# klemens-floege/oneprot

Measured on AMD Instinct MI355X. Metric: protein-pairs/sec/node (seq+struct-token, L=512, ESM-2-150M), higher is better.
Workload: dtype bf16; 1 GPU; cfg-2: seq<->struct_token sub-step, facebook/esm2_t30_150M_UR50D / facebook/esm2_t30_150M_UR50D, L=512, 256 pairs/GPU per modality, global batch 256, output_dim 1024, CLIP local_loss+gather_with_grad, L1 0.01, Adam 1e-3, clip 1.0, sequence encoder frozen (reference default), random-init weights; global_batch=256, seq_len=512, parallelism=dp1, frozen_sequence_encoder=True

## Files before the change

include/oneprot_hip.h:

```cpp
#ifndef ONEPROT_HIP_H
#define ONEPROT_HIP_H
#include <stddef.h>
#include <stdint.h>
#ifdef __cplusplus
extern "C" {
#endif

int oneprot_abi_version(void);

int oneprot_esm_embed_fwd(const int64_t* ids, const float* table, float* x, float* row_scale, int B, int L, int d, int vocab,
                          int pad_id, int mask_id, int token_dropout, void* stream);
size_t oneprot_esm_embed_bwd_workspace(int T, int d, int vocab);
int oneprot_esm_embed_bwd(const int64_t* ids, const float* dx, const float* row_scale, float* dtable, void* workspace, int B, int L, int d,
                          int vocab, int pad_id, int mask_id, int token_dropout, int accumulate, void* stream);
int oneprot_bert_embed_fwd(const int64_t* ids, const float* word, const float* pos, const float* type0, const float* gamma, const float* beta,
                           float* x_f32, void* x_bf16, int B, int L, int d, int vocab, float eps, void* stream);

int oneprot_layernorm_fwd(const void* x, int x_is_bf16, const float* gamma, const float* beta, void* y_bf16, float* y_f32, float* mean,
                          float* rstd, int64_t T, int d, float eps, void* stream);
size_t oneprot_layernorm_bwd_workspace(int d);
int oneprot_layernorm_bwd(const void* dy, int dy_mode, const float* wrow, int L, const void* x, int x_is_bf16, const float* gamma,
                          const float* mean, const float* rstd, const float* add_to, float* dx, void* dx_bf16 ,
                          float* dgamma, float* dbeta, void* workspace, int64_t T, int d, int accumulate_param_grads, void* stream);
int oneprot_lnpool_fwd(const float* x, const int64_t* ids, int pad_id, const float* gamma, const float* beta, float* pooled, float* mean,
// ... 33 lines not shown
int oneprot_sched_late_draws(const void* sched_ws);
int64_t oneprot_sched_epoch(const void* sched_ws);
int oneprot_gemm_resid_ln8_eligible(int64_t M, int N, int K);
int oneprot_gemm_resid_ln8_error(const void* sched_ws);
int oneprot_gemm_resid_ln8_error_clear(void* sched_ws, void* stream);
void oneprot_gemm_resid_ln8_poll_bound(int polls);
int oneprot_gemm_bf16_nt_resid_ln8(const void* A, const void* W, int64_t M, int N, int K, int lda, int ldb, const float* bias, const float* resid,
                                   float* x_out, const float* gamma, const float* beta, float eps, void* h_bf16, float* stats, void* sched_ws,
                                   size_t sched_ws_bytes, void* stream);
void oneprot_gemm_ln_form(int form);
int oneprot_gemm_ln_form_get(void);
void oneprot_gemm_force_shape(int shape);
void oneprot_gemm_tune(int sup_m, int sup_n);
size_t oneprot_gemm_bf16_tn_workspace(int N, int K);
void oneprot_gemm_tn_variant(int v);
void oneprot_cu_reserve(int cus);
int oneprot_gemm_bf16_tn(const void* dY, const void* X, int64_t M, int N, int K, int ldy, int ldx, float* dW, float* dbias, void* workspace,
                         size_t workspace_bytes, int accumulate, void* stream);
int oneprot_sgemm(const float* A, const float* B, float* C, int M, int N, int K, int transA, int b_is_kn, float alpha, int accumulate, void* stream);

int oneprot_attn_fwd(const void* q, const void* k, const void* v, const float* key_bias, void* ctx, float* lse, int B, int H, int L, int hd,
                     void* stream);
size_t oneprot_attn_bwd_workspace(int B, int H, int L);
int oneprot_attn_bwd(const void* q, const void* k, const void* v, const float* key_bias, const void* ctx, const void* dctx, const float* lse,
                     const float* rope_cos, const float* rope_sin, float q_scale, void* dqkv, void* workspace, int B, int H, int L, int hd,
                     void* stream);
int oneprot_attn_fwd_dropout(const void* q, const void* k, const void* v, const float* key_bias, void* ctx, float* lse, int B, int H, int L, int hd,
                             float p, uint64_t seed, uint64_t stream_id, void* stream);
int oneprot_attn_bwd_dropout(const void* q, const void* k, const void* v, const float* key_bias, const void* ctx, const void* dctx, const float* lse,
                             const float* rope_cos, const float* rope_sin, float q_scale, void* dqkv, void* workspace, int B, int H, int L, int hd,
                             float p, uint64_t seed, uint64_t stream_id, void* stream);
int oneprot_attn_dropout_keep(void* keep, int B, int H, int L, float p, uint64_t seed, uint64_t stream_id, void* stream);
void oneprot_attn_force_bwd_path(int path);
void oneprot_attn_force_fwd_path(int path);

int oneprot_gelu_f32(const float* x, float* y, int64_t n, void* stream);
int oneprot_gelu_bwd_f32(const float* x, const float* dy, float* dx, int64_t n, void* stream);
int oneprot_l2norm_fwd(const float* x, float* y, float* inv_norm, int R, int D, float scale, void* stream);
int oneprot_l2norm_bwd(const float* y, const float* dy, const float* inv_norm, float* dx, int R, int D, float scale, float l1_coef, void* stream);
int oneprot_ce_fwd_bwd(float* logits, float* loss_sum, float* row_loss_ws , int R, int C, int label_offset, float row_weight, void* stream);
int oneprot_siglip_fwd_bwd(float* logits, float* loss_sum, float* row_loss_ws , int B, float logit_bias, int negative_only, void* stream);
int oneprot_siglip_fwd_bwd_dev(float* logits, float* loss_sum, float* row_loss_ws , int B, const float* logit_bias_dev, int negative_only, void* stream);
int oneprot_diag_rank(const float* logits, int* rank_row, int* rank_col, int N, void* stream);
int oneprot_abs_sum(const float* x, float* out_sum, void* workspace , int64_t n, float coef, void* stream);

int oneprot_dot_f32(const float* x, const float* y, float* out_sum, void* workspace , int64_t n, float coef, void* stream);

int oneprot_l1_bwd(const float* x, float* dx, int64_t n, float coef, const float* upstream, int accumulate, void* stream);
int oneprot_scale_by_device_scalar(float* x, int64_t n, const float* s, void* stream);
int oneprot_key_padding_bias(const int64_t* ids, float* bias, int64_t n, int pad_id, void* stream);

int oneprot_dropout_bf16(const void* x, void* y, int64_t n, float p, uint64_t seed, uint64_t stream_id, void* stream);
int oneprot_dropout_f32(const float* x, float* y, int64_t n, float p, uint64_t seed, uint64_t stream_id, void* stream);
int oneprot_dropout_add_f32(const float* x, const float* resid, float* y, int64_t n, float p, uint64_t seed, uint64_t stream_id, void* stream);
int oneprot_dropout_add_layernorm_fwd(const float* x, const float* resid, float* s_out, const float* gamma, const float* beta, void* y_bf16, float* y_f32,
                                      float* mean, float* rstd, int64_t T, int d, float eps, float p, uint64_t seed, uint64_t stream_id, void* stream);
int oneprot_dropout_bwd_add_bf16(const void* dy, void* dx, int64_t n, float p, uint64_t seed, uint64_t stream_id, void* stream);
int oneprot_dropout_bwd_add_f32(const void* dy, float* dx, int64_t n, float p, uint64_t seed, uint64_t stream_id, void* stream);

size_t oneprot_sumsq_workspace(void);
int oneprot_sumsq(const float* x, int64_t n, float* sumsq, void* workspace, void* stream);
int oneprot_clip_coef(const float* sumsq, float max_norm, float* coef, float* norm_out, const void* sched_ws , void* stream);
int oneprot_adam_step(float* p, const float* g, float* m, float* v, int64_t n, float lr, float beta1, float beta2, float eps, float weight_decay,
                      int step, const float* grad_scale, void* stream);

int oneprot_cast_f32_to_bf16(const float* src, void* dst, int64_t n, void* stream);
// ... 31 lines not shown
```

oneprot_amd/csrc/attention.hip:

```cpp
#include "common.h"
#include "sched_ws.h"
#include "../../include/oneprot_hip.h"
#include <float.h>
#include <atomic>
void* dynamic_tiles_workspace();

#define LOG2E 1.4426950408889634f
#define KC 256
#define RESCALE_THR 10.0f

template <int HD> struct Cfg {
  static constexpr int HDP = HD < 32 ? 32 : HD;
  static constexpr int NCH = HDP / 8;
  static constexpr int KSTEPS = HD / 16;
  static constexpr int DBLK = HDP / 32;
  static constexpr int ROWB = HDP * 2;
};

template <int HDP> __device__ __forceinline__ int swz(int row, int chunk) {
  return HDP == 32 ? (chunk ^ ((row >> 2) & 3)) : (chunk ^ ((row >> 1) & 7));
}

template <int HD> struct TileRegs { u32x4 v[KC * Cfg<HD>::NCH / 256]; };
template <int HD>
// ... 1312 lines not shown
  if (!q || !k || !v || !ctx || B <= 0 || H <= 0 || L <= 0) return OP_EINVAL;
  hipStream_t s = (hipStream_t)stream;
  if (g_attn_fwd_path != 0) {
    switch (hd) {
      case 16: return launch_fwd_nomax<16>(q, k, v, key_bias, ctx, lse, B, H, L, s);
      case 32: return launch_fwd_nomax<32>(q, k, v, key_bias, ctx, lse, B, H, L, s);
      case 64: return launch_fwd_nomax<64>(q, k, v, key_bias, ctx, lse, B, H, L, s);
      default: return OP_EINVAL;
    }
  }
  switch (hd) {
    case 16: return launch_fwd<16>(q, k, v, key_bias, ctx, lse, B, H, L, s);
    case 32: return launch_fwd<32>(q, k, v, key_bias, ctx, lse, B, H, L, s);
    case 64: return launch_fwd<64>(q, k, v, key_bias, ctx, lse, B, H, L, s);
    default: return OP_EINVAL;
  }
}

extern "C" int oneprot_attn_fwd_dropout(const void* q, const void* k, const void* v, const float* key_bias, void* ctx, float* lse, int B, int H, int L, int hd, float p,
                                        uint64_t seed, uint64_t stream_id, void* stream) {
  AttnDrop dr;
  if (!q || !k || !v || !ctx || B <= 0 || H <= 0 || L <= 0 || attn_drop_make(p, seed, stream_id, dr) != OP_OK) return OP_EINVAL;
  hipStream_t s = (hipStream_t)stream;
  switch (hd) {
    case 16: return launch_fwd_dropout<16>(q, k, v, key_bias, ctx, lse, B, H, L, dr, s);
    case 32: return launch_fwd_dropout<32>(q, k, v, key_bias, ctx, lse, B, H, L, dr, s);
    case 64: return launch_fwd_dropout<64>(q, k, v, key_bias, ctx, lse, B, H, L, dr, s);
    default: return OP_EINVAL;
  }
}

template <int HD>
__device__ __forceinline__ void unrope_store(f32x16 (&acc)[Cfg<HD>::DBLK], const float* __restrict__ cosT, const float* __restrict__ sinT, int pos, int h,
                                             float scale, bool rope, bf16_t* dst) {
  typedef Cfg<HD> C;
  constexpr int HALF = HD / 2;
#pragma unroll
  for (int d = 0; d < C::DBLK; ++d)
#pragma unroll
    for (int g = 0; g < 4; ++g) {
      const int dd = 32 * d + 8 * g + 4 * h;
      if (dd >= HD) continue;
      float o[4];
      if (rope) {
        const bool lo = dd < HALF;
        const int jj = lo ? dd : dd - HALF;
        const float4 c = *reinterpret_cast<const float4*>(cosT + (size_t)pos * HALF + jj);
        const float4 sn = *reinterpret_cast<const float4*>(sinT + (size_t)pos * HALF + jj);
        float own[4], par[4];
#pragma unroll
        for (int e = 0; e < 4; ++e) own[e] = acc[d][4 * g + e];
        if (HD == 64) {
#pragma unroll
          for (int e = 0; e < 4; ++e) par[e] = acc[C::DBLK - 1 - d][4 * g + e];
        } else if (HD == 32) {
#pragma unroll
          for (int e = 0; e < 4; ++e) par[e] = acc[0][4 * (g ^ 2) + e];
        } else {
#pragma unroll
          for (int e = 0; e < 4; ++e) par[e] = acc[0][4 * (g ^ 1) + e];
        }
        const float cv[4] = {c.x, c.y, c.z, c.w}, sv[4] = {sn.x, sn.y, sn.z, sn.w};
#pragma unroll
        for (int e = 0; e < 4; ++e) o[e] = (own[e] * cv[e] + (lo ? par[e] : -par[e]) * sv[e]) * scale;
      } else {
#pragma unroll
        for (int e = 0; e < 4; ++e) o[e] = acc[d][4 * g + e] * scale;
      }
      u32x2 w; w.x = pack2bf(o[0], o[1]); w.y = pack2bf(o[2], o[3]);
      *reinterpret_cast<u32x2*>(dst + dd) = w;
    }
}

template <int HD, bool DROP = false>
__global__ void __launch_bounds__(256, 2) k_attn_bwd_dq(const bf16_t* __restrict__ q, const bf16_t* __restrict__ k, const bf16_t* __restrict__ v,
                                                     const float* __restrict__ key_bias, const bf16_t* __restrict__ ctx, const bf16_t* __restrict__ dctx,
                                                     const float* __restrict__ lse, float* __restrict__ delta, const float* __restrict__ cosT, const float* __restrict__ sinT,
                                                     float q_scale, bf16_t* __restrict__ dqkv, int B, int H, int L, int nqb, const AttnDrop dr = AttnDrop{0u, 0u, 0u, 1.0f}) {
  typedef Cfg<HD> C;
  extern __shared__ __attribute__((aligned(16))) unsigned char smem[];
  unsigned char* sK = smem;
// ... 380 lines not shown
          f32x16 a0[1] = {dq};
          if (qidx < L && !(abl & 16)) unrope_store<HD>(a0, cosT, sinT, qidx, h, q_scale, cosT != nullptr, dqkv + ((size_t)b * L + qidx) * (3 * dm) + head * HD);
        }
        i = i + 1 == nblk ? 0 : i + 1;
        ticket += visits(i);
      }
      tbase += nwaves;
    }
  }
  if (active && !(abl & 32)) {
    f32x16 a1[1] = {adk}, a2[1] = {adv};
#pragma unroll
    for (int which = 0; which < 2; ++which) {
      bf16_t* img = reinterpret_cast<bf16_t*>(sT + r * 64);
      if (which == 0) unrope_store<HD>(a1, cosT, sinT, kidx < L ? kidx : 0, h, 0.6931471805599453f, cosT != nullptr, img);
      else unrope_store<HD>(a2, cosT, sinT, 0, h, 1.0f, false, img);
      asm volatile("s_waitcnt lgkmcnt(0)" ::: "memory");
#pragma unroll
      for (int it = 0; it < 2; ++it) {
        const int idx = lane + 64 * it, row = idx >> 2, ch = idx & 3;
        const u32x4 w = *reinterpret_cast<const u32x4*>(sT + row * 64 + ch * 16);
        if (key0 + row < L && ch < HD / 8)
          *reinterpret_cast<u32x4*>(dqkv + ((size_t)b * L + key0 + row) * (3 * dm) + (which + 1) * dm + head * HD + ch * 8) = w;
      }
      asm volatile("s_waitcnt lgkmcnt(0)" ::: "memory");
    }
  }
}

#ifndef BWD64_PRIO
#define BWD64_PRIO 1
#endif
#ifdef BWD64_STAMP
__device__ unsigned long long g_bwd64_stamps[8 * 16 * 8];
extern "C" int oneprot_attn_debug_bwd64_stamps(unsigned long long* host_out) {
  return hipMemcpyFromSymbol(host_out, HIP_SYMBOL(g_bwd64_stamps), sizeof(g_bwd64_stamps)) == hipSuccess ? 0 : -2;
}
#define BWD64_T(i)                                                                                   \
  do {                                                                                               \
    __builtin_amdgcn_sched_barrier(0);                                                               \
    unsigned long long t_;                                                                           \
    asm volatile("s_memtime %0\n\ts_waitcnt lgkmcnt(0)" : "=s"(t_)::"memory");                        \
    if (lane == 0 && blockIdx.x == 2053) g_bwd64_stamps[(wave * 16 + (blk0 + t)) * 8 + (i)] = t_;   \
    __builtin_amdgcn_sched_barrier(0);                                                               \
  } while (0)
#else
#define BWD64_T(i) do { } while (0)
#endif

template <int HD>
__global__ void __launch_bounds__(512, 1) k_attn_bwd_fused64(const bf16_t* __restrict__ q, const bf16_t* __restrict__ k, const bf16_t* __restrict__ v,
                                                           const float* __restrict__ key_bias, const bf16_t* __restrict__ ctx, const bf16_t* __restrict__ dctx,
                                                           const float* __restrict__ lse, const float* __restrict__ cosT, const float* __restrict__ sinT,
                                                           float q_scale, bf16_t* __restrict__ dqkv, int B, int H, int L, int dph) {
  typedef Cfg<HD> C;
  typedef FusedLds<HD> F;
  extern __shared__ __attribute__((aligned(16))) unsigned char smem[];
  unsigned char* sQ = smem;
  unsigned char* sdO = sQ + F::TILE;
  u32x4* sQE = reinterpret_cast<u32x4*>(sdO + F::TILE);
  lds_vint* sTicket = (lds_vint*)LDS_PTR(sdO + F::TILE + (F::ROWS + 1) * 16);
  float* sdQ = reinterpret_cast<float*>(sdO + F::TILE + F::QE);
  const int lane = threadIdx.x & 63, wave = __builtin_amdgcn_readfirstlane(threadIdx.x >> 6), h = lane >> 5, r = lane & 31;
  unsigned char* sT = reinterpret_cast<unsigned char*>(sdQ) + F::DQ + wave * 2 * F::SLAB;
  const int dm = H * HD;
  const int nbh = B * H, per_xcd = (nbh + 7) >> 3;
  const int bh = (int)(blockIdx.x & 7) * per_xcd + (int)(blockIdx.x >> 3);
  if (bh >= nbh) return;
  const int b = bh / H, head = bh - b * H;
  const int key0 = wave * 64;
  const bool active = key0 < L;

  u32x4 kr[4], vr[4];
#pragma unroll
  for (int it = 0; it < 4; ++it) {
    const int idx = lane + 64 * it, row = idx >> 2, ch = idx & 3;
    const u32x4 z = {0u, 0u, 0u, 0u};
    kr[it] = z; vr[it] = z;
    if (key0 + row < L && ch < HD / 8) {
      kr[it] = *reinterpret_cast<const u32x4*>(k + ((size_t)bh * L + key0 + row) * HD + ch * 8);
      vr[it] = *reinterpret_cast<const u32x4*>(v + ((size_t)bh * L + key0 + row) * HD + ch * 8);
    }
  }
  float bias_k[2];
#pragma unroll
  for (int kb = 0; kb < 2; ++kb) {
    const int kidx = key0 + 32 * kb + r;
    bias_k[kb] = kidx < L ? (key_bias ? key_bias[(size_t)b * L + kidx] : 0.f) : -INFINITY;
  }
  {
    const bf16_t* qrow0 = q + (size_t)bh * L * HD;
    const bf16_t* dorow0 = dctx + (size_t)b * L * dm + head * HD;
    const bf16_t* orow0 = ctx + (size_t)b * L * dm + head * HD;
    const int nrows = (L + 31) & ~31;
    {
      u32x4 rq[4], rdo[4], ro[4];
      float rl[4];
#pragma unroll
      for (int it = 0; it < 4; ++it) {
        const int idx = threadIdx.x + 512 * it, row = idx >> 2, ch = idx & 3;
        const u32x4 z = {0u, 0u, 0u, 0u};
        rq[it] = z; rdo[it] = z; ro[it] = z; rl[it] = 0.f;
        if (row < L) {
          if (ch < HD / 8) {
            rq[it] = *reinterpret_cast<const u32x4*>(qrow0 + (size_t)row * HD + ch * 8);
            rdo[it] = *reinterpret_cast<const u32x4*>(dorow0 + (size_t)row * dm + ch * 8);
            ro[it] = *reinterpret_cast<const u32x4*>(orow0 + (size_t)row * dm + ch * 8);
          }
          if (ch == 0) rl[it] = lse[(size_t)bh * L + row];
        }
      }
#pragma unroll
      for (int it = 0; it < 4; ++it) {
        const int idx = threadIdx.x + 512 * it, row = idx >> 2, ch = idx & 3;
        float part = dot8_bf16(rdo[it], ro[it]);
        part += __shfl_xor(part, 1, 64);
        part += __shfl_xor(part, 2, 64);
        if (row < nrows) {
          const int off = row * 64 + (swz<32>(row, ch) << 4);
          *reinterpret_cast<u32x4*>(sQ + off) = rq[it];
          *reinterpret_cast<u32x4*>(sdO + off) = rdo[it];
          if (ch == 0) {
            u32x4 e;
            unsigned w01, w2;
            split3_bf16(row < L ? -rl[it] * LOG2E : -1.0e30f, w01, w2);
            e.x = w01; e.y = w2 | 0x3F800000u;
            split3_bf16(row < L ? -part : 0.f, w01, w2);
            e.z = w01; e.w = w2;
            sQE[row] = e;
          }
        }
      }
    }
    const u32x4 z = {0u, 0u, 0u, 0u};
    if (threadIdx.x == 0) sQE[F::ROWS] = z;
    if (threadIdx.x < FQB) sTicket[threadIdx.x] = 0;
  }

  bf8_t kf[2][C::KSTEPS], vf[2][C::KSTEPS], ktf[2][2];
  {
#pragma unroll
    for (int it = 0; it < 4; ++it) {
      const int idx = lane + 64 * it, row = idx >> 2, ch = idx & 3;
      *reinterpret_cast<u32x4*>(sT + row * 64 + (swz<32>(row, ch) << 4)) = kr[it];
    }
#pragma unroll
    for (int kb = 0; kb < 2; ++kb) {
#pragma unroll
      for (int st = 0; st < C::KSTEPS; ++st) kf[kb][st] = rd_row<HD>(sT + kb * F::SLAB, r, st, h);
      ktf[kb][0] = rd_tr<HD>(sT + kb * F::SLAB, 0, 0, 0, lane);
      ktf[kb][1] = rd_tr<HD>(sT + kb * F::SLAB, 0, 1, 0, lane);
    }
    asm volatile("s_waitcnt lgkmcnt(0)" ::: "memory");
#pragma unroll
    for (int it = 0; it < 4; ++it) {
      const int idx = lane + 64 * it, row = idx >> 2, ch = idx & 3;
      *reinterpret_cast<u32x4*>(sT + row * 64 + (swz<32>(row, ch) << 4)) = vr[it];
    }
#pragma unroll
    for (int kb = 0; kb < 2; ++kb)
#pragma unroll
      for (int st = 0; st < C::KSTEPS; ++st) vf[kb][st] = rd_row<HD>(sT + kb * F::SLAB, r, st, h);
    asm volatile("s_waitcnt lgkmcnt(0)" ::: "memory");
  }
  unsigned ky[2];
#pragma unroll
  for (int kb = 0; kb < 2; ++kb) ky[kb] = h == 0 ? (0x3F80u | (pack2bf(bias_k[kb], 0.f) << 16)) : 0u;
  const unsigned hm = h == 0 ? 0x3F803F80u : 0u;
  f32x16 adk[2] = {zero16(), zero16()}, adv[2] = {zero16(), zero16()};

  const int sw = (r >> 2) & 3;
  int row_off[C::KSTEPS];
#pragma unroll
  for (int st = 0; st < C::KSTEPS; ++st) row_off[st] = r * 64 + (((2 * st + h) ^ sw) << 4);
  int tr_off[2][2];
  {
    const int g = lane >> 4, i = lane & 15;
    const int col = 16 * (g & 1) + 4 * (i & 3);
#pragma unroll
    for (int sb = 0; sb < 2; ++sb) {
      const int r0 = 16 * sb + 4 * h + (i >> 2), r1 = r0 + 8;
      tr_off[sb][0] = r0 * 64 + (swz<32>(r0, col >> 3) << 4) + (col & 7) * 2;
      tr_off[sb][1] = r1 * 64 + (swz<32>(r1, col >> 3) << 4) + (col & 7) * 2;
    }
  }
  const int wr_off = r * 64 + 8 * h;
  auto tr_frag = [&](const unsigned char* base, int sb) -> bf8_t {
    const s16x4 a = __builtin_amdgcn_ds_read_tr16_b64_v4i16((__attribute__((address_space(3))) s16x4*)(base + tr_off[sb][0]));
    const s16x4 c = __builtin_amdgcn_ds_read_tr16_b64_v4i16((__attribute__((address_space(3))) s16x4*)(base + tr_off[sb][1]));
    s16x8 o;
    o[0] = a[0]; o[1] = a[1]; o[2] = a[2]; o[3] = a[3]; o[4] = c[0]; o[5] = c[1]; o[6] = c[2]; o[7] = c[3];
    return __builtin_bit_cast(bf8_t, o);
  };
  __syncthreads();

  if (wave >= 4 && dph < 900) for (int i = 0; i < dph; ++i) __builtin_amdgcn_s_sleep(1);
  if (active) {
    const int nkw = (L + 63) >> 6;
    const int nqb = (L + 31) >> 5;
    int p_i = -1, p_turn = 0, p_ticket = 0, p_qblk = 0;
    auto dq_mfmas = [&]() -> f32x16 {
      f32x16 dq = MFMA32(ktf[0][0], tr_frag(sT, 0), zero16());
      dq = MFMA32(ktf[1][0], tr_frag(sT + F::SLAB, 0), dq);
      dq = MFMA32(ktf[0][1], tr_frag(sT, 1), dq);
      dq = MFMA32(ktf[1][1], tr_frag(sT + F::SLAB, 1), dq);
      return dq;
    };
    auto dq_commit = [&](f32x16& dq) {
#ifdef ONEPROT_ATTN_ABLATE
      if (dph == 900 || dph == 901) { asm volatile("" :: "v"(dq[0]), "v"(dq[5]), "v"(dq[10]), "v"(dq[15])); return; }
#endif
      if (lane == 0)
        while (sTicket[p_i] != p_turn) __builtin_amdgcn_s_sleep(1);
      asm volatile("" ::: "memory");
      float4* drow = reinterpret_cast<float4*>(sdQ + (p_i * 32 + r) * F::DQP + 4 * h);
      if (p_ticket != 0) {
#pragma unroll
        for (int g = 0; g < 4; ++g) {
          const float4 o = drow[2 * g];
          dq[4 * g] += o.x; dq[4 * g + 1] += o.y; dq[4 * g + 2] += o.z; dq[4 * g + 3] += o.w;
        }
      }
      if (p_ticket != nkw - 1) {
#pragma unroll
        for (int g = 0; g < 4; ++g) drow[2 * g] = make_float4(dq[4 * g], dq[4 * g + 1], dq[4 * g + 2], dq[4 * g + 3]);
      }
      asm volatile("" ::: "memory");
      if (lane == 0) sTicket[p_i] = p_turn + 1;
      if (p_ticket == nkw - 1) {
// ... 72 lines not shown
          const u32x4 w0 = __builtin_bit_cast(u32x4, dsf[0]), w1 = __builtin_bit_cast(u32x4, dsf[1]);
          u32x2 g0 = {w0.x, w0.y}, g1 = {w0.z, w0.w}, g2 = {w1.x, w1.y}, g3 = {w1.z, w1.w};
          unsigned char* slab = sT + kb * F::SLAB;
          *reinterpret_cast<u32x2*>(slab + wr_off + ((0 ^ sw) << 4)) = g0;
          *reinterpret_cast<u32x2*>(slab + wr_off + ((1 ^ sw) << 4)) = g1;
          *reinterpret_cast<u32x2*>(slab + wr_off + ((2 ^ sw) << 4)) = g2;
          *reinterpret_cast<u32x2*>(slab + wr_off + ((3 ^ sw) << 4)) = g3;
        };
        chains(1);
        vector_part(0);
#pragma unroll
        for (int n = 0; n < 6; ++n) {
          __builtin_amdgcn_sched_group_barrier(0x008, 1, 0);
          __builtin_amdgcn_sched_group_barrier(0x002, 9, 0);
        }
        __builtin_amdgcn_sched_barrier(0);
        matrix_part(0);
        vector_part(1);
#pragma unroll
        for (int n = 0; n < 4; ++n) {
          __builtin_amdgcn_sched_group_barrier(0x008, 1, 1);
          __builtin_amdgcn_sched_group_barrier(0x002, 14, 1);
        }
        __builtin_amdgcn_sched_barrier(0);
        matrix_part(1);
        asm volatile("" ::: "memory");
        BWD64_T(3);
        p_i = i; p_turn = tbase + ticket; p_ticket = ticket; p_qblk = qblk;
        i = i + 1 == nblk ? 0 : i + 1;
        ticket += visits(i);
      }
      tbase += nkw;
    }
    if (p_i >= 0) {
      f32x16 dql = dq_mfmas();
      dq_commit(dql);
    }
  }
  if (active) {
#pragma unroll
    for (int kb = 0; kb < 2; ++kb) {
      const int kidx = key0 + 32 * kb + r;
      f32x16 a1[1] = {adk[kb]}, a2[1] = {adv[kb]};
      unsigned char* slab = sT + kb * F::SLAB;
#pragma unroll
      for (int which = 0; which < 2; ++which) {
        bf16_t* img = reinterpret_cast<bf16_t*>(slab + r * 64);
        if (which == 0) unrope_store<HD>(a1, cosT, sinT, kidx < L ? kidx : 0, h, 0.6931471805599453f, cosT != nullptr, img);
        else unrope_store<HD>(a2, cosT, sinT, 0, h, 1.0f, false, img);
        asm volatile("s_waitcnt lgkmcnt(0)" ::: "memory");
#pragma unroll
        for (int it = 0; it < 2; ++it) {
          const int idx = lane + 64 * it, row = idx >> 2, ch = idx & 3;
          const u32x4 w = *reinterpret_cast<const u32x4*>(slab + row * 64 + ch * 16);
          if (key0 + 32 * kb + row < L && ch < HD / 8)
            *reinterpret_cast<u32x4*>(dqkv + ((size_t)b * L + key0 + 32 * kb + row) * (3 * dm) + (which + 1) * dm + head * HD + ch * 8) = w;
        }
        asm volatile("s_waitcnt lgkmcnt(0)" ::: "memory");
      }
    }
  }
}

static int g_attn_bwd_path = -1;
extern "C" void oneprot_attn_force_bwd_path(int path) { g_attn_bwd_path = path < 0 ? -1 : (path > 2 ? 2 : path); }
#ifdef ONEPROT_ATTN_ABLATE
static int g_attn_bwd_ablate = 0;
extern "C" void oneprot_attn_debug_ablate(int mask) { g_attn_bwd_ablate = mask; }
#else
static constexpr int g_attn_bwd_ablate = 0;
#endif

template <int HD>
static int launch_bwd(const void* q, const void* k, const void* v, const float* key_bias, const void* ctx, const void* dctx, const float* lse, float* delta,
                      const float* cosT, const float* sinT, float q_scale, void* dqkv, int B, int H, int L, hipStream_t s) {
  if constexpr (HD <= 32) {
    const int path = g_attn_bwd_path >= 0 ? g_attn_bwd_path : (L <= 288 ? 0 : (L <= 416 ? 1 : 2));
    if (L <= 512 && path != 0) {
      static int fused_ok = -1;
      if (fused_ok < 0)
        fused_ok = hipFuncSetAttribute((const void*)k_attn_bwd_fused<HD>, hipFuncAttributeMaxDynamicSharedMemorySize, FusedLds<HD>::TOTAL) == hipSuccess ? 1 : 0;
      if (!fused_ok) { (void)hipGetLastError(); if (g_attn_bwd_path > 0) return OP_EINVAL; }
      else if (path == 2) {
        static int f64_ok = -1;
        if (f64_ok < 0)
          f64_ok = hipFuncSetAttribute((const void*)k_attn_bwd_fused64<HD>, hipFuncAttributeMaxDynamicSharedMemorySize, FusedLds<HD>::TOTAL) == hipSuccess ? 1 : 0;
        if (!f64_ok) { (void)hipGetLastError(); if (g_attn_bwd_path > 0) return OP_EINVAL; }
        else {
        hipLaunchKernelGGL(k_attn_bwd_fused64<HD>, dim3(((B * H + 7) / 8) * 8), dim3(512), FusedLds<HD>::TOTAL, s, (const bf16_t*)q, (const bf16_t*)k, (const bf16_t*)v, key_bias,
                           (const bf16_t*)ctx, (const bf16_t*)dctx, lse, cosT, sinT, q_scale, (bf16_t*)dqkv, B, H, L, g_attn_bwd_ablate);
        return launch_status();
        }
      } else {
      hipLaunchKernelGGL(k_attn_bwd_fused<HD>, dim3(((B * H + 7) / 8) * 8), dim3(1024), FusedLds<HD>::TOTAL, s, (const bf16_t*)q, (const bf16_t*)k, (const bf16_t*)v, key_bias,
                         (const bf16_t*)ctx, (const bf16_t*)dctx, lse, cosT, sinT, q_scale, (bf16_t*)dqkv, B, H, L, g_attn_bwd_ablate);
      return launch_status();
      }
    }
  }
  const int nb = (L + 127) / 128;
  const int nbh8 = ((B * H + 7) / 8) * 8;
  const size_t lds_q = (size_t)2 * KC * Cfg<HD>::ROWB + (KC + 1) * 16;
  const size_t lds_kv = (size_t)2 * KC * Cfg<HD>::ROWB + (KC + 1) * 16;
  hipLaunchKernelGGL(k_attn_bwd_dq<HD>, dim3(nbh8 * nb), dim3(256), lds_q, s, (const bf16_t*)q, (const bf16_t*)k, (const bf16_t*)v, key_bias,
                     (const bf16_t*)ctx, (const bf16_t*)dctx, lse, delta, cosT, sinT, q_scale, (bf16_t*)dqkv, B, H, L, nb);
  hipLaunchKernelGGL(k_attn_bwd_dkv<HD>, dim3(nbh8 * nb), dim3(256), lds_kv, s, (const bf16_t*)q, (const bf16_t*)k, (const bf16_t*)v, key_bias,
                     (const bf16_t*)dctx, lse, (const float*)delta, cosT, sinT, (bf16_t*)dqkv, B, H, L, nb);
  return launch_status();
}

extern "C" size_t oneprot_attn_bwd_workspace(int B, int H, int L) { return (size_t)B * H * L * sizeof(float); }

template <int HD>
static int launch_bwd_dropout(const void* q, const void* k, const void* v, const float* key_bias, const void* ctx, const void* dctx, const float* lse, float* delta,
                              const float* cosT, const float* sinT, float q_scale, void* dqkv, int B, int H, int L, const AttnDrop& dr, hipStream_t s) {
  const int nb = (L + 127) / 128;
  const int nbh8 = ((B * H + 7) / 8) * 8;
  const size_t lds = (size_t)2 * KC * Cfg<HD>::ROWB + (KC + 1) * 16;
  hipLaunchKernelGGL((k_attn_bwd_dq<HD, true>), dim3(nbh8 * nb), dim3(256), lds, s, (const bf16_t*)q, (const bf16_t*)k, (const bf16_t*)v, key_bias,
                     (const bf16_t*)ctx, (const bf16_t*)dctx, lse, delta, cosT, sinT, q_scale, (bf16_t*)dqkv, B, H, L, nb, dr);
  hipLaunchKernelGGL((k_attn_bwd_dkv<HD, true>), dim3(nbh8 * nb), dim3(256), lds, s, (const bf16_t*)q, (const bf16_t*)k, (const bf16_t*)v, key_bias,
// ... 374 lines not shown
```

oneprot_amd/csrc/check_resources.py:

```python
#!/usr/bin/env python3
import re
import subprocess
import sys

RULES = [
    (r"^void g8::k_gemm8<", 0),
    (r"^void k_gemm_tn8<", 0),
    (r"^void gln::k_gemm_ln", 0),
    (r"^void k_attn_fwd3<", 0),
    (r"^void k_attn_fwd3w<", 0),
    (r"^void k_attn_fwd2<", 16),
    (r"^void k_attn_bwd_fused<\(int\)32>", 0),
    (r"^void k_attn_bwd_fused64<\(int\)32>", 0),
    (r"^void k_layernorm_(fwd|bwd)", 0),
]


def parse(text):
    out = {}
    cur = None
    for line in text.splitlines():
        m = re.search(r"Function Name: (\S+)", line)
        if m:
            cur = m.group(1)
            out[cur] = {}
            continue
        for key, pat in (("vgpr", r"\bVGPRs: (\d+)"), ("agpr", r"AGPRs: (\d+)"), ("scratch", r"ScratchSize \[bytes/lane\]: (\d+)"), ("occ", r"Occupancy \[waves/SIMD\]: (\d+)")):
            m = re.search(pat, line)
            if m and cur:
                out[cur][key] = int(m.group(1))
    return out


def demangle(names):
    try:
        p = subprocess.run(["c++filt"], input="\n".join(names), capture_output=True, text=True, check=True)
        return dict(zip(names, p.stdout.splitlines()))
    except Exception:
        return {n: n for n in names}


def main():
    args = [a for a in sys.argv[1:] if not a.startswith("--")]
    text = "".join(open(a).read() for a in args) if args else sys.stdin.read()
    kernels = parse(text)
    names = demangle(list(kernels))
# ... 16 lines not shown
```

oneprot_amd/hip.py:

```python
import ctypes
import os
from ctypes import c_float, c_int, c_int64, c_size_t, c_void_p

import torch

_HERE = os.path.dirname(os.path.abspath(__file__))
LIB_PATH = os.environ.get("ONEPROT_HIP_LIB") or os.path.join(_HERE, "liboneprot_hip.so")

ABI_VERSION = 7
EPI_BF16, EPI_F32, EPI_BIAS_GELU, EPI_BIAS_RESID, EPI_QKV_ROPE, EPI_GELU_BWD = range(6)
LOG2E = 1.4426950408889634


class HipLibraryMissing(RuntimeError):
    pass


class HipKernelError(RuntimeError):
    pass


P, I, L64, F, SZ = c_void_p, c_int, c_int64, c_float, c_size_t
U64 = ctypes.c_uint64

# ... 15 lines not shown
    "oneprot_layernorm_bwd": (I, [P, I, P, I, P, I, P, P, P, P, P, P, P, P, P, L64, I, I, P]),
    "oneprot_lnpool_fwd": (I, [P, P, I, P, P, P, P, P, P, P, P, I, I, I, F, I, P]),
    "oneprot_gemm_bf16_nt": (I, [P, P, L64, I, I, I, I, I, P, P, P, P, P, P, P, F, I, I, I, P]),
    "oneprot_gemm_ln_pack_weight": (I, [P, P, I, I, P]),
    "oneprot_gemm_bf16_nt_resid_ln": (I, [P, P, L64, I, I, I, P, P, P, P, P, F, P, P, P, P]),
    "oneprot_sched_workspace_bytes": (SZ, [L64]),
    "oneprot_alloc_uncached": (I, [ctypes.POINTER(c_void_p), SZ]),
    "oneprot_free_uncached": (I, [P]),
    "oneprot_sched_workspace_init": (I, [P, SZ, P]),
    "oneprot_dynamic_tiles": (None, [P, SZ]),
    "oneprot_sched_late_draws": (I, [P]),
    "oneprot_sched_epoch": (L64, [P]),
    "oneprot_gemm_bf16_nt_resid_ln8": (I, [P, P, L64, I, I, I, I, P, P, P, P, P, F, P, P, P, SZ, P]),
    "oneprot_gemm_resid_ln8_eligible": (I, [L64, I, I]),
    "oneprot_gemm_resid_ln8_error": (I, [P]),
    "oneprot_gemm_resid_ln8_error_clear": (I, [P, P]),
    "oneprot_gemm_resid_ln8_poll_bound": (None, [I]),
    "oneprot_gemm_ln_form": (None, [I]),
    "oneprot_gemm_ln_form_get": (I, []),
    "oneprot_gemm_force_shape": (None, [I]),
    "oneprot_gemm_tune": (None, [I, I]),
    "oneprot_gemm_bf16_tn_workspace": (SZ, [I, I]),
    "oneprot_gemm_tn_variant": (None, [I]),
    "oneprot_cu_reserve": (None, [I]),
    "oneprot_gemm_bf16_tn": (I, [P, P, L64, I, I, I, I, P, P, P, SZ, I, P]),
    "oneprot_sgemm": (I, [P, P, P, I, I, I, I, I, F, I, P]),
    "oneprot_attn_fwd": (I, [P, P, P, P, P, P, I, I, I, I, P]),
    "oneprot_attn_fwd_dropout": (I, [P, P, P, P, P, P, I, I, I, I, F, U64, U64, P]),
    "oneprot_attn_dropout_keep": (I, [P, I, I, I, F, U64, U64, P]),
    "oneprot_attn_bwd_dropout": (I, [P, P, P, P, P, P, P, P, P, F, P, P, I, I, I, I, F, U64, U64, P]),
    "oneprot_attn_bwd_workspace": (SZ, [I, I, I]),
    "oneprot_attn_bwd": (I, [P, P, P, P, P, P, P, P, P, F, P, P, I, I, I, I, P]),
    "oneprot_attn_force_bwd_path": (None, [I]),
    "oneprot_attn_force_fwd_path": (None, [I]),
    "oneprot_gelu_f32": (I, [P, P, L64, P]),
    "oneprot_gelu_bwd_f32": (I, [P, P, P, L64, P]),
    "oneprot_l2norm_fwd": (I, [P, P, P, I, I, F, P]),
    "oneprot_l2norm_bwd": (I, [P, P, P, P, I, I, F, F, P]),
    "oneprot_ce_fwd_bwd": (I, [P, P, P, I, I, I, F, P]),
    "oneprot_siglip_fwd_bwd": (I, [P, P, P, I, F, I, P]),
    "oneprot_siglip_fwd_bwd_dev": (I, [P, P, P, I, P, I, P]),
    "oneprot_diag_rank": (I, [P, P, P, I, P]),
    "oneprot_abs_sum": (I, [P, P, P, L64, F, P]),
    "oneprot_dot_f32": (I, [P, P, P, P, L64, F, P]),
    "oneprot_l1_bwd": (I, [P, P, L64, F, P, I, P]),
    "oneprot_scale_by_device_scalar": (I, [P, L64, P, P]),
    "oneprot_dropout_bf16": (I, [P, P, L64, F, U64, U64, P]),
    "oneprot_dropout_bwd_add_bf16": (I, [P, P, L64, F, U64, U64, P]),
    "oneprot_dropout_bwd_add_f32": (I, [P, P, L64, F, U64, U64, P]),
    "oneprot_dropout_f32": (I, [P, P, L64, F, U64, U64, P]),
    "oneprot_dropout_add_f32": (I, [P, P, P, L64, F, U64, U64, P]),
    "oneprot_dropout_add_layernorm_fwd": (I, [P, P, P, P, P, P, P, P, P, L64, I, F, F, U64, U64, P]),
    "oneprot_key_padding_bias": (I, [P, P, L64, I, P]),
    "oneprot_sumsq_workspace": (SZ, []),
    "oneprot_sumsq": (I, [P, L64, P, P, P]),
    "oneprot_clip_coef": (I, [P, F, P, P, P, P]),
    "oneprot_adam_step": (I, [P, P, P, P, L64, F, F, F, F, F, I, P, P]),
    "oneprot_cast_f32_to_bf16": (I, [P, P, L64, P]),
    "oneprot_transpose_cast_f32_to_bf16": (I, [P, P, I, I, P]),
    "oneprot_transpose_cast_f32_to_bf16_batched": (I, [P, P, I, I, L64, L64, I, P]),
    "oneprot_colsum_workspace": (SZ, [I]),
    "oneprot_colsum_bf16": (I, [P, P, P, L64, I, I, P]),
    "oneprot_esm_embed_packed_fwd": (I, [P, P, P, P, P, P, P, P, P, I, I, I, I, I, I, I, I, I, I, P]),
    "oneprot_esm_embed_packed_bwd": (I, [P, P, P, P, P, I, I, I, I, I, I, I, P]),
    "oneprot_attn_varlen_fwd": (I, [P, P, P, P, P, I, P, P, I, I, I, I, P]),
    "oneprot_attn_varlen_bwd_workspace": (SZ, [I, I]),
# ... 199 lines not shown
```

Baseline: 1185 protein-pairs/sec/node.

## Make fused attention backward persistent and prefetch next head's inputs during dK/dV store

Adds a persistent variant of the fused 64-key attention backward kernel, launched with one block per CU slot per XCD, where each block loops over (batch, head) pairs. While it stores dK/dV for the current head, it issues global loads of K/V/Q/dO/O/LSE for the next head, and it preloads the rope cos/sin values before the final dQ commit. The aim is to hide load latency and avoid per-block launch and prologue cost. The trade-offs are higher register pressure, which the spill check now guards, and possible load imbalance when the head count does not divide evenly across slots. The persistent form is the default, with a switch to fall back to the old launch.

```diff
diff --git a/include/oneprot_hip.h b/include/oneprot_hip.h
--- a/include/oneprot_hip.h
+++ b/include/oneprot_hip.h
@@ -89,6 +89,8 @@
                              float p, uint64_t seed, uint64_t stream_id, void* stream);
 int oneprot_attn_dropout_keep(void* keep, int B, int H, int L, float p, uint64_t seed, uint64_t stream_id, void* stream);
 void oneprot_attn_force_bwd_path(int path);
+void oneprot_attn_bwd64_form(int form);
+int oneprot_attn_bwd64_form_get(void);
 void oneprot_attn_force_fwd_path(int path);
 
 int oneprot_gelu_f32(const float* x, float* y, int64_t n, void* stream);
diff --git a/oneprot_amd/csrc/attention.hip b/oneprot_amd/csrc/attention.hip
--- a/oneprot_amd/csrc/attention.hip
+++ b/oneprot_amd/csrc/attention.hip
@@ -1368,7 +1368,7 @@
 
 template <int HD>
 __device__ __forceinline__ void unrope_store(f32x16 (&acc)[Cfg<HD>::DBLK], const float* __restrict__ cosT, const float* __restrict__ sinT, int pos, int h,
-                                             float scale, bool rope, bf16_t* dst) {
+                                             float scale, bool rope, bf16_t* dst, const float4* pre_cos = nullptr, const float4* pre_sin = nullptr) {
   typedef Cfg<HD> C;
   constexpr int HALF = HD / 2;
 #pragma unroll
@@ -1381,8 +1381,8 @@
       if (rope) {
         const bool lo = dd < HALF;
         const int jj = lo ? dd : dd - HALF;
-        const float4 c = *reinterpret_cast<const float4*>(cosT + (size_t)pos * HALF + jj);
-        const float4 sn = *reinterpret_cast<const float4*>(sinT + (size_t)pos * HALF + jj);
+        const float4 c = pre_cos ? pre_cos[HD == 32 ? (g & 1) : 0] : *reinterpret_cast<const float4*>(cosT + (size_t)pos * HALF + jj);
+        const float4 sn = pre_sin ? pre_sin[HD == 32 ? (g & 1) : 0] : *reinterpret_cast<const float4*>(sinT + (size_t)pos * HALF + jj);
         float own[4], par[4];
 #pragma unroll
         for (int e = 0; e < 4; ++e) own[e] = acc[d][4 * g + e];
@@ -1829,27 +1829,45 @@
 #define BWD64_PRIO 1
 #endif
 #ifdef BWD64_STAMP
+#ifndef BWD64_STAMP_SLAB
+#define BWD64_STAMP_SLAB 8
+#endif
 __device__ unsigned long long g_bwd64_stamps[8 * 16 * 8];
+__device__ unsigned long long g_bwd64_phases[2 * 8 * 8];
 extern "C" int oneprot_attn_debug_bwd64_stamps(unsigned long long* host_out) {
   return hipMemcpyFromSymbol(host_out, HIP_SYMBOL(g_bwd64_stamps), sizeof(g_bwd64_stamps)) == hipSuccess ? 0 : -2;
+}
+extern "C" int oneprot_attn_debug_bwd64_phases(unsigned long long* host_out) {
+  return hipMemcpyFromSymbol(host_out, HIP_SYMBOL(g_bwd64_phases), sizeof(g_bwd64_phases)) == hipSuccess ? 0 : -2;
 }
 #define BWD64_T(i)                                                                                   \
   do {                                                                                               \
     __builtin_amdgcn_sched_barrier(0);                                                               \
     unsigned long long t_;                                                                           \
     asm volatile("s_memtime %0\n\ts_waitcnt lgkmcnt(0)" : "=s"(t_)::"memory");                        \
-    if (lane == 0 && blockIdx.x == 2053) g_bwd64_stamps[(wave * 16 + (blk0 + t)) * 8 + (i)] = t_;   \
+    if (lane == 0 && stamp_slab == 0) g_bwd64_stamps[(wave * 16 + (blk0 + t)) * 8 + (i)] = t_;      \
+    __builtin_amdgcn_sched_barrier(0);                                                               \
+  } while (0)
+#define BWD64_P(i, drain_vm)                                                                         \
+  do {                                                                                               \
+    __builtin_amdgcn_sched_barrier(0);                                                               \
+    unsigned long long t_;                                                                           \
+    if (drain_vm) asm volatile("s_waitcnt vmcnt(0)" ::: "memory");                                  \
+    asm volatile("s_memtime %0\n\ts_waitcnt lgkmcnt(0)" : "=s"(t_)::"memory");                        \
+    if (lane == 0 && (stamp_slab == 0 || stamp_slab == 1)) g_bwd64_phases[(stamp_slab * 8 + wave) * 8 + (i)] = t_; \
     __builtin_amdgcn_sched_barrier(0);                                                               \
   } while (0)
 #else
 #define BWD64_T(i) do { } while (0)
-#endif
-
-template <int HD>
-__global__ void __launch_bounds__(512, 1) k_attn_bwd_fused64(const bf16_t* __restrict__ q, const bf16_t* __restrict__ k, const bf16_t* __restrict__ v,
-                                                           const float* __restrict__ key_bias, const bf16_t* __restrict__ ctx, const bf16_t* __restrict__ dctx,
-                                                           const float* __restrict__ lse, const float* __restrict__ cosT, const float* __restrict__ sinT,
-                                                           float q_scale, bf16_t* __restrict__ dqkv, int B, int H, int L, int dph) {
+#define BWD64_P(i, drain_vm) do { } while (0)
+#endif
+
+__device__ __forceinline__ int here(int x) { asm volatile("" : "+v"(x)); return x; }
+template <int HD, bool PERSIST>
+__device__ __forceinline__ void attn_bwd_fused64_body(const bf16_t* __restrict__ q, const bf16_t* __restrict__ k, const bf16_t* __restrict__ v,
+                                                      const float* __restrict__ key_bias, const bf16_t* __restrict__ ctx, const bf16_t* __restrict__ dctx,
+                                                      const float* __restrict__ lse, const float* __restrict__ cosT, const float* __restrict__ sinT,
+                                                      float q_scale, bf16_t* __restrict__ dqkv, int B, int H, int L, int dph) {
   typedef Cfg<HD> C;
   typedef FusedLds<HD> F;
   extern __shared__ __attribute__((aligned(16))) unsigned char smem[];
@@ -1862,54 +1880,95 @@
   unsigned char* sT = reinterpret_cast<unsigned char*>(sdQ) + F::DQ + wave * 2 * F::SLAB;
   const int dm = H * HD;
   const int nbh = B * H, per_xcd = (nbh + 7) >> 3;
-  const int bh = (int)(blockIdx.x & 7) * per_xcd + (int)(blockIdx.x >> 3);
-  if (bh >= nbh) return;
-  const int b = bh / H, head = bh - b * H;
+  const int xcd0 = (int)(blockIdx.x & 7) * per_xcd, nslot = PERSIST ? (int)(gridDim.x >> 3) : per_xcd;
+  int slot = (int)(blockIdx.x >> 3);
+  int bh = xcd0 + slot;
+  if (slot >= per_xcd || bh >= nbh) return;
   const int key0 = wave * 64;
   const bool active = key0 < L;
-
-  u32x4 kr[4], vr[4];
-#pragma unroll
-  for (int it = 0; it < 4; ++it) {
-    const int idx = lane + 64 * it, row = idx >> 2, ch = idx & 3;
-    const u32x4 z = {0u, 0u, 0u, 0u};
-    kr[it] = z; vr[it] = z;
-    if (key0 + row < L && ch < HD / 8) {
-      kr[it] = *reinterpret_cast<const u32x4*>(k + ((size_t)bh * L + key0 + row) * HD + ch * 8);
-      vr[it] = *reinterpret_cast<const u32x4*>(v + ((size_t)bh * L + key0 + row) * HD + ch * 8);
-    }
-  }
-  float bias_k[2];
-#pragma unroll
-  for (int kb = 0; kb < 2; ++kb) {
-    const int kidx = key0 + 32 * kb + r;
-    bias_k[kb] = kidx < L ? (key_bias ? key_bias[(size_t)b * L + kidx] : 0.f) : -INFINITY;
-  }
+#ifdef BWD64_STAMP
+  int stamp_slab = PERSIST ? (blockIdx.x == 53 ? -BWD64_STAMP_SLAB : -1000000) : (blockIdx.x == 2053 ? 0 : -1000000);
+#endif
+  BWD64_P(0, false);
+
+  u32x4 kr[4], vr[4], rq[4], rdo[4], ro[4];
+  float rl[4], bias_k[2];
+  auto request_kv_rows = [&](const int sbh) {
+    const int sb = sbh / H, shead = sbh - sb * H;
+    const int tid = here(threadIdx.x), lane = tid & 63, r = lane & 31;
+    const unsigned char* kbase = reinterpret_cast<const unsigned char*>(k + (size_t)sbh * L * HD);
+    const unsigned char* vbase = reinterpret_cast<const unsigned char*>(v + (size_t)sbh * L * HD);
+#pragma unroll
+    for (int it = 0; it < 4; ++it) {
+      const int idx = lane + 64 * it, row = min(key0 + (idx >> 2), L - 1), ch = idx & (HD / 8 - 1);
+      const unsigned off = (unsigned)(row * HD + ch * 8) * 2u;
+      kr[it] = *reinterpret_cast<const u32x4*>(kbase + off);
+      vr[it] = *reinterpret_cast<const u32x4*>(vbase + off);
+    }
+    const float* brow = key_bias ? key_bias + (size_t)sb * L : lse + (size_t)sbh * L;
+#pragma unroll
+    for (int kb = 0; kb < 2; ++kb) bias_k[kb] = brow[(unsigned)min(key0 + 32 * kb + r, L - 1)];
+  };
+  auto request_q_rows = [&](const int sbh) {
+    const int sb = sbh / H, shead = sbh - sb * H;
+    const int tid = here(threadIdx.x);
+    const unsigned char* qbase = reinterpret_cast<const unsigned char*>(q + (size_t)sbh * L * HD);
+    const unsigned char* dobase = reinterpret_cast<const unsigned char*>(dctx + (size_t)sb * L * dm + shead * HD);
+    const unsigned char* obase = reinterpret_cast<const unsigned char*>(ctx + (size_t)sb * L * dm + shead * HD);
+    const float* lrow = lse + (size_t)sbh * L;
+#pragma unroll
+    for (int it = 0; it < 4; ++it) {
+      const int idx = tid + 512 * it, row = min(idx >> 2, L - 1), ch = idx & (HD / 8 - 1);
+      const unsigned qoff = (unsigned)(row * HD + ch * 8) * 2u, ooff = (unsigned)(row * dm + ch * 8) * 2u;
+      rq[it] = *reinterpret_cast<const u32x4*>(qbase + qoff);
+      rdo[it] = *reinterpret_cast<const u32x4*>(dobase + ooff);
+      ro[it] = *reinterpret_cast<const u32x4*>(obase + ooff);
+      rl[it] = lrow[(unsigned)row];
+    }
+  };
+  request_kv_rows(bh);
+  request_q_rows(bh);
+  BWD64_P(1, false);
+
+  const int sw = (r >> 2) & 3;
+  int row_off[C::KSTEPS];
+#pragma unroll
+  for (int st = 0; st < C::KSTEPS; ++st) row_off[st] = r * 64 + (((2 * st + h) ^ sw) << 4);
+  int tr_off[2][2];
   {
-    const bf16_t* qrow0 = q + (size_t)bh * L * HD;
-    const bf16_t* dorow0 = dctx + (size_t)b * L * dm + head * HD;
-    const bf16_t* orow0 = ctx + (size_t)b * L * dm + head * HD;
+    const int g = lane >> 4, i = lane & 15;
+    const int col = 16 * (g & 1) + 4 * (i & 3);
+#pragma unroll
+    for (int sb = 0; sb < 2; ++sb) {
+      const int r0 = 16 * sb + 4 * h + (i >> 2), r1 = r0 + 8;
+      tr_off[sb][0] = r0 * 64 + (swz<32>(r0, col >> 3) << 4) + (col & 7) * 2;
+      tr_off[sb][1] = r1 * 64 + (swz<32>(r1, col >> 3) << 4) + (col & 7) * 2;
+    }
+  }
+  const int wr_off = r * 64 + 8 * h;
+  const unsigned hm = h == 0 ? 0x3F803F80u : 0u;
+  auto tr_frag = [&](const unsigned char* base, int sb) -> bf8_t {
+    const s16x4 a = __builtin_amdgcn_ds_read_tr16_b64_v4i16((__attribute__((address_space(3))) s16x4*)(base + tr_off[sb][0]));
+    const s16x4 c = __builtin_amdgcn_ds_read_tr16_b64_v4i16((__attribute__((address_space(3))) s16x4*)(base + tr_off[sb][1]));
+    s16x8 o;
+    o[0] = a[0]; o[1] = a[1]; o[2] = a[2]; o[3] = a[3]; o[4] = c[0]; o[5] = c[1]; o[6] = c[2]; o[7] = c[3];
+    return __builtin_bit_cast(bf8_t, o);
+  };
+
+  for (;;) {
+  const int b = bh / H, head = bh - b * H;
+  BWD64_P(2, true);
+  {
+    const int tid = here(threadIdx.x);
     const int nrows = (L + 31) & ~31;
     {
-      u32x4 rq[4], rdo[4], ro[4];
-      float rl[4];
 #pragma unroll
       for (int it = 0; it < 4; ++it) {
-        const int idx = threadIdx.x + 512 * it, row = idx >> 2, ch = idx & 3;
-        const u32x4 z = {0u, 0u, 0u, 0u};
-        rq[it] = z; rdo[it] = z; ro[it] = z; rl[it] = 0.f;
-        if (row < L) {
-          if (ch < HD / 8) {
-            rq[it] = *reinterpret_cast<const u32x4*>(qrow0 + (size_t)row * HD + ch * 8);
-            rdo[it] = *reinterpret_cast<const u32x4*>(dorow0 + (size_t)row * dm + ch * 8);
-            ro[it] = *reinterpret_cast<const u32x4*>(orow0 + (size_t)row * dm + ch * 8);
-          }
-          if (ch == 0) rl[it] = lse[(size_t)bh * L + row];
-        }
-      }
-#pragma unroll
-      for (int it = 0; it < 4; ++it) {
-        const int idx = threadIdx.x + 512 * it, row = idx >> 2, ch = idx & 3;
+        const int idx = tid + 512 * it, row = idx >> 2, ch = idx & 3;
+        if (!(row < L && ch < HD / 8)) {
+          const u32x4 z = {0u, 0u, 0u, 0u};
+          rq[it] = z; rdo[it] = z; ro[it] = z;
+        }
         float part = dot8_bf16(rdo[it], ro[it]);
         part += __shfl_xor(part, 1, 64);
         part += __shfl_xor(part, 2, 64);
@@ -1930,15 +1989,20 @@
       }
     }
     const u32x4 z = {0u, 0u, 0u, 0u};
-    if (threadIdx.x == 0) sQE[F::ROWS] = z;
-    if (threadIdx.x < FQB) sTicket[threadIdx.x] = 0;
+    if (tid == 0) sQE[F::ROWS] = z;
+    if (tid < FQB) sTicket[tid] = 0;
   }
 
   bf8_t kf[2][C::KSTEPS], vf[2][C::KSTEPS], ktf[2][2];
   {
+    const int lane = here(threadIdx.x) & 63, h = lane >> 5, r = lane & 31;
 #pragma unroll
     for (int it = 0; it < 4; ++it) {
       const int idx = lane + 64 * it, row = idx >> 2, ch = idx & 3;
+      if (!(key0 + row < L && ch < HD / 8)) {
+        const u32x4 z = {0u, 0u, 0u, 0u};
+        kr[it] = z; vr[it] = z;
+      }
       *reinterpret_cast<u32x4*>(sT + row * 64 + (swz<32>(row, ch) << 4)) = kr[it];
     }
 #pragma unroll
@@ -1962,36 +2026,16 @@
   }
   unsigned ky[2];
 #pragma unroll
-  for (int kb = 0; kb < 2; ++kb) ky[kb] = h == 0 ? (0x3F80u | (pack2bf(bias_k[kb], 0.f) << 16)) : 0u;
-  const unsigned hm = h == 0 ? 0x3F803F80u : 0u;
+  for (int kb = 0; kb < 2; ++kb) {
+    const float bk = key0 + 32 * kb + r < L ? (key_bias ? bias_k[kb] : 0.f) : -INFINITY;
+    ky[kb] = h == 0 ? (0x3F80u | (pack2bf(bk, 0.f) << 16)) : 0u;
+  }
   f32x16 adk[2] = {zero16(), zero16()}, adv[2] = {zero16(), zero16()};
-
-  const int sw = (r >> 2) & 3;
-  int row_off[C::KSTEPS];
-#pragma unroll
-  for (int st = 0; st < C::KSTEPS; ++st) row_off[st] = r * 64 + (((2 * st + h) ^ sw) << 4);
-  int tr_off[2][2];
-  {
-    const int g = lane >> 4, i = lane & 15;
-    const int col = 16 * (g & 1) + 4 * (i & 3);
-#pragma unroll
-    for (int sb = 0; sb < 2; ++sb) {
-      const int r0 = 16 * sb + 4 * h + (i >> 2), r1 = r0 + 8;
-      tr_off[sb][0] = r0 * 64 + (swz<32>(r0, col >> 3) << 4) + (col & 7) * 2;
-      tr_off[sb][1] = r1 * 64 + (swz<32>(r1, col >> 3) << 4) + (col & 7) * 2;
-    }
-  }
-  const int wr_off = r * 64 + 8 * h;
-  auto tr_frag = [&](const unsigned char* base, int sb) -> bf8_t {
-    const s16x4 a = __builtin_amdgcn_ds_read_tr16_b64_v4i16((__attribute__((address_space(3))) s16x4*)(base + tr_off[sb][0]));
-    const s16x4 c = __builtin_amdgcn_ds_read_tr16_b64_v4i16((__attribute__((address_space(3))) s16x4*)(base + tr_off[sb][1]));
-    s16x8 o;
-    o[0] = a[0]; o[1] = a[1]; o[2] = a[2]; o[3] = a[3]; o[4] = c[0]; o[5] = c[1]; o[6] = c[2]; o[7] = c[3];
-    return __builtin_bit_cast(bf8_t, o);
-  };
   __syncthreads();
+  BWD64_P(3, false);
 
   if (wave >= 4 && dph < 900) for (int i = 0; i < dph; ++i) __builtin_amdgcn_s_sleep(1);
+  float4 ecos[2][HD / 16], esin[2][HD / 16];
   if (active) {
     const int nkw = (L + 63) >> 6;
     const int nqb = (L + 31) >> 5;
@@ -2130,38 +2174,99 @@
       }
       tbase += nkw;
     }
+    {
+      const float* ct = cosT ? cosT : reinterpret_cast<const float*>(q + (size_t)bh * L * HD);
+      const float* st = cosT ? sinT : ct;
+      const int lane = here(threadIdx.x) & 63, h = lane >> 5, r = lane & 31;
+#pragma unroll
+      for (int kb = 0; kb < 2; ++kb) {
+        const int kidx = key0 + 32 * kb + r, pos = kidx < L ? kidx : 0;
+#pragma unroll
+        for (int j = 0; j < HD / 16; ++j) {
+          ecos[kb][j] = *reinterpret_cast<const float4*>(ct + (size_t)pos * (HD / 2) + 8 * j + 4 * h);
+          esin[kb][j] = *reinterpret_cast<const float4*>(st + (size_t)pos * (HD / 2) + 8 * j + 4 * h);
+        }
+      }
+    }
     if (p_i >= 0) {
       f32x16 dql = dq_mfmas();
       dq_commit(dql);
     }
   }
-  if (active) {
-#pragma unroll
-    for (int kb = 0; kb < 2; ++kb) {
-      const int kidx = key0 + 32 * kb + r;
-      f32x16 a1[1] = {adk[kb]}, a2[1] = {adv[kb]};
-      unsigned char* slab = sT + kb * F::SLAB;
-#pragma unroll
-      for (int which = 0; which < 2; ++which) {
-        bf16_t* img = reinterpret_cast<bf16_t*>(slab + r * 64);
-        if (which == 0) unrope_store<HD>(a1, cosT, sinT, kidx < L ? kidx : 0, h, 0.6931471805599453f, cosT != nullptr, img);
-        else unrope_store<HD>(a2, cosT, sinT, 0, h, 1.0f, false, img);
-        asm volatile("s_waitcnt lgkmcnt(0)" ::: "memory");
-#pragma unroll
-        for (int it = 0; it < 2; ++it) {
-          const int idx = lane + 64 * it, row = idx >> 2, ch = idx & 3;
-          const u32x4 w = *reinterpret_cast<const u32x4*>(slab + row * 64 + ch * 16);
-          if (key0 + 32 * kb + row < L && ch < HD / 8)
-            *reinterpret_cast<u32x4*>(dqkv + ((size_t)b * L + key0 + 32 * kb + row) * (3 * dm) + (which + 1) * dm + head * HD + ch * 8) = w;
-        }
-        asm volatile("s_waitcnt lgkmcnt(0)" ::: "memory");
-      }
-    }
-  }
+  BWD64_P(4, false);
+  slot += nslot;
+  const int bh_next = xcd0 + slot;
+  const bool more = PERSIST && slot < per_xcd && bh_next < nbh;
+  auto store_dkv = [&](const int kb, const int which) {
+    const int lane = here(threadIdx.x) & 63, h = lane >> 5, r = lane & 31;
+    const int kidx = key0 + 32 * kb + r;
+    unsigned char* slab = sT + kb * F::SLAB;
+    bf16_t* img = reinterpret_cast<bf16_t*>(slab + r * 64);
+    if (which == 0) {
+      f32x16 a1[1] = {adk[kb]};
+      unrope_store<HD>(a1, cosT, sinT, kidx < L ? kidx : 0, h, 0.6931471805599453f, cosT != nullptr, img, ecos[kb], esin[kb]);
+    } else {
+      f32x16 a2[1] = {adv[kb]};
+      unrope_store<HD>(a2, cosT, sinT, 0, h, 1.0f, false, img);
+    }
+    asm volatile("s_waitcnt lgkmcnt(0)" ::: "memory");
+#pragma unroll
+    for (int it = 0; it < 2; ++it) {
+      const int idx = lane + 64 * it, row = idx >> 2, ch = idx & 3;
+      const u32x4 w = *reinterpret_cast<const u32x4*>(slab + row * 64 + ch * 16);
+      if (key0 + 32 * kb + row < L && ch < HD / 8)
+        *reinterpret_cast<u32x4*>(dqkv + ((size_t)b * L + key0 + 32 * kb + row) * (3 * dm) + (which + 1) * dm + head * HD + ch * 8) = w;
+    }
+    asm volatile("s_waitcnt lgkmcnt(0)" ::: "memory");
+  };
+  if constexpr (PERSIST) {
+    if (more) {
+      request_kv_rows(bh_next);
+      request_q_rows(bh_next);
+      BWD64_P(7, false);
+    } else {
+      const u32x4 z = {0u, 0u, 0u, 0u};
+#pragma unroll
+      for (int it = 0; it < 4; ++it) { kr[it] = z; vr[it] = z; rq[it] = z; rdo[it] = z; ro[it] = z; rl[it] = 0.f; }
+      bias_k[0] = bias_k[1] = 0.f;
+    }
+  }
+  if (active) { store_dkv(0, 0); store_dkv(1, 0); store_dkv(0, 1); store_dkv(1, 1); }
+  BWD64_P(5, false);
+  if (!more) {
+    BWD64_P(6, false);
+    break;
+  }
+  __syncthreads();
+  BWD64_P(6, false);
+#ifdef BWD64_STAMP
+  ++stamp_slab;
+#endif
+  BWD64_P(0, false);
+  bh = bh_next;
+  }
+}
+
+template <int HD>
+__global__ void __launch_bounds__(512, 1) k_attn_bwd_fused64(const bf16_t* __restrict__ q, const bf16_t* __restrict__ k, const bf16_t* __restrict__ v,
+                                                           const float* __restrict__ key_bias, const bf16_t* __restrict__ ctx, const bf16_t* __restrict__ dctx,
+                                                           const float* __restrict__ lse, const float* __restrict__ cosT, const float* __restrict__ sinT,
+                                                           float q_scale, bf16_t* __restrict__ dqkv, int B, int H, int L, int dph) {
+  attn_bwd_fused64_body<HD, false>(q, k, v, key_bias, ctx, dctx, lse, cosT, sinT, q_scale, dqkv, B, H, L, dph);
+}
+template <int HD>
+__global__ void __launch_bounds__(512, 1) k_attn_bwd_fused64p(const bf16_t* __restrict__ q, const bf16_t* __restrict__ k, const bf16_t* __restrict__ v,
+                                                            const float* __restrict__ key_bias, const bf16_t* __restrict__ ctx, const bf16_t* __restrict__ dctx,
+                                                            const float* __restrict__ lse, const float* __restrict__ cosT, const float* __restrict__ sinT,
+                                                            float q_scale, bf16_t* __restrict__ dqkv, int B, int H, int L, int dph) {
+  attn_bwd_fused64_body<HD, true>(q, k, v, key_bias, ctx, dctx, lse, cosT, sinT, q_scale, dqkv, B, H, L, dph);
 }
 
 static int g_attn_bwd_path = -1;
 extern "C" void oneprot_attn_force_bwd_path(int path) { g_attn_bwd_path = path < 0 ? -1 : (path > 2 ? 2 : path); }
+static int g_attn_bwd64_form = 0;
+extern "C" void oneprot_attn_bwd64_form(int form) { g_attn_bwd64_form = form == 1 ? 1 : 0; }
+extern "C" int oneprot_attn_bwd64_form_get(void) { return g_attn_bwd64_form; }
 #ifdef ONEPROT_ATTN_ABLATE
 static int g_attn_bwd_ablate = 0;
 extern "C" void oneprot_attn_debug_ablate(int mask) { g_attn_bwd_ablate = mask; }
@@ -2182,9 +2287,24 @@
       else if (path == 2) {
         static int f64_ok = -1;
         if (f64_ok < 0)
-          f64_ok = hipFuncSetAttribute((const void*)k_attn_bwd_fused64<HD>, hipFuncAttributeMaxDynamicSharedMemorySize, FusedLds<HD>::TOTAL) == hipSuccess ? 1 : 0;
+          f64_ok = hipFuncSetAttribute((const void*)k_attn_bwd_fused64<HD>, hipFuncAttributeMaxDynamicSharedMemorySize, FusedLds<HD>::TOTAL) == hipSuccess &&
+                   hipFuncSetAttribute((const void*)k_attn_bwd_fused64p<HD>, hipFuncAttributeMaxDynamicSharedMemorySize, FusedLds<HD>::TOTAL) == hipSuccess ? 1 : 0;
         if (!f64_ok) { (void)hipGetLastError(); if (g_attn_bwd_path > 0) return OP_EINVAL; }
-        else {
+        else if (g_attn_bwd64_form == 0) {
+          static int n_cu = 0;
+          if (n_cu <= 0) {
+            int dev = 0; hipDeviceProp_t prop;
+            if (hipGetDevice(&dev) != hipSuccess || hipGetDeviceProperties(&prop, dev) != hipSuccess) { (void)hipGetLastError(); return OP_ELAUNCH; }
+            n_cu = prop.multiProcessorCount;
+          }
+          const int per_xcd = (B * H + 7) / 8;
+          int nslot = n_cu / 8;
+          if (nslot < 1) nslot = 1;
+          if (nslot > per_xcd) nslot = per_xcd;
+          hipLaunchKernelGGL(k_attn_bwd_fused64p<HD>, dim3(8 * nslot), dim3(512), FusedLds<HD>::TOTAL, s, (const bf16_t*)q, (const bf16_t*)k, (const bf16_t*)v, key_bias,
+                             (const bf16_t*)ctx, (const bf16_t*)dctx, lse, cosT, sinT, q_scale, (bf16_t*)dqkv, B, H, L, g_attn_bwd_ablate);
+          return launch_status();
+        } else {
         hipLaunchKernelGGL(k_attn_bwd_fused64<HD>, dim3(((B * H + 7) / 8) * 8), dim3(512), FusedLds<HD>::TOTAL, s, (const bf16_t*)q, (const bf16_t*)k, (const bf16_t*)v, key_bias,
                            (const bf16_t*)ctx, (const bf16_t*)dctx, lse, cosT, sinT, q_scale, (bf16_t*)dqkv, B, H, L, g_attn_bwd_ablate);
         return launch_status();
diff --git a/oneprot_amd/csrc/check_resources.py b/oneprot_amd/csrc/check_resources.py
--- a/oneprot_amd/csrc/check_resources.py
+++ b/oneprot_amd/csrc/check_resources.py
@@ -12,6 +12,7 @@
     (r"^void k_attn_fwd2<", 16),
     (r"^void k_attn_bwd_fused<\(int\)32>", 0),
     (r"^void k_attn_bwd_fused64<\(int\)32>", 0),
+    (r"^void k_attn_bwd_fused64p<(\(int\))?(16|32)>", 0),
     (r"^void k_layernorm_(fwd|bwd)", 0),
 ]
 
diff --git a/oneprot_amd/hip.py b/oneprot_amd/hip.py
--- a/oneprot_amd/hip.py
+++ b/oneprot_amd/hip.py
@@ -71,6 +71,8 @@
     "oneprot_attn_bwd_workspace": (SZ, [I, I, I]),
     "oneprot_attn_bwd": (I, [P, P, P, P, P, P, P, P, P, F, P, P, I, I, I, I, P]),
     "oneprot_attn_force_bwd_path": (None, [I]),
+    "oneprot_attn_bwd64_form": (None, [I]),
+    "oneprot_attn_bwd64_form_get": (I, []),
     "oneprot_attn_force_fwd_path": (None, [I]),
     "oneprot_gelu_f32": (I, [P, P, L64, P]),
     "oneprot_gelu_bwd_f32": (I, [P, P, P, L64, P]),
```

Measured after the change: 1191 protein-pairs/sec/node, median of 6. No clear change (+0.5%).
